# ziqin-h/GIVEPose

Measured on AMD Instinct MI355X. Metric: images/sec PoseNet fwd, bs=64 256x256 fp16, 1/2/4/8 MI355X; % MFMA roofline, higher is better.
Workload: dtype f16

## Files before the change

givepose_amd/_lib.py:

```python
import ctypes
import os
from ctypes import POINTER, Structure, c_char_p, c_double, c_float, c_int, c_long, c_void_p

_HERE = os.path.dirname(os.path.abspath(__file__))
LIB_PATH = os.environ.get("GP_LIB_PATH") or os.path.join(_HERE, "libgivepose_hip.so")

ABI_VERSION = 328
GP_F32, GP_F16, GP_F64 = 0, 1, 2
ACT_NONE, ACT_GELU, ACT_RELU, ACT_LRELU = 0, 1, 2, 3
EPI_NONE, EPI_GELU, EPI_RELU, EPI_LRELU, EPI_SCALE_RES, EPI_RES_RELU, EPI_LNFOLD_GELU = 0, 1, 2, 3, 4, 5, 6
ROT_6D, ROT_6D_Y, ROT_6D_Z, ROT_QUAT, ROT_EULER = 0, 1, 2, 3, 4
KC_GEMM, KC_DCNV3, KC_DWCONV_LN, KC_NORM, KC_ELEMENTWISE, KC_SMALL, KC_COUNT = 0, 1, 2, 3, 4, 5, 6
KC_NAMES = ["gemm", "dcnv3", "dwconv_ln", "norm", "elementwise", "small"]


class GemmDesc(Structure):
    _fields_ = [("X", c_void_p), ("W", c_void_p), ("bias", c_void_p), ("gamma", c_void_p), ("residual", c_void_p),
                ("C", c_void_p), ("workspace", c_void_p),
                ("M", c_int), ("N", c_int), ("K", c_int), ("ldx", c_int), ("ldc", c_int), ("ldres", c_int),
                ("epilogue", c_int), ("out_f32", c_int), ("splitk", c_int),
                ("B", c_int), ("H", c_int), ("Win", c_int), ("Cin", c_int), ("KH", c_int), ("KW", c_int),
                ("stride", c_int), ("pad", c_int), ("Ho", c_int), ("Wo", c_int), ("dtype", c_int),
                ("gn_partial", c_void_p), ("gn_groups", c_int), ("gn_hw", c_int), ("variant", c_int),
                ("ln_stats", c_void_p), ("ln_colsum", c_void_p), ("ln_nslab", c_int), ("ln_eps", c_float),
                ("co_scheduled", c_int), ("prefetch", c_void_p), ("prefetch_bytes", c_long),
                ("split_shift", c_int), ("x_plane_stride", c_long), ("w_plane_stride", c_long),
                ("out_planes", c_int), ("c_plane_stride", c_long),
                ("residual_f32", c_int), ("c16", c_void_p), ("ldc16", c_int), ("gn_rows", c_int)]


_P = c_void_p
PROTOTYPES = {
    "gp_last_error": ([], c_char_p),
    "gp_version": ([], c_int),
    "gp_device_info": ([POINTER(c_int), c_char_p, c_int], c_int),
    "gp_dcnv3_forward": ([_P, _P, _P, _P] + [c_int] * 9 + [c_float] + [c_int] * 7 + [_P], c_int),
    "gp_dcnv3_forward_any": ([_P] * 4 + [c_int] * 13 + [c_float] + [c_int] * 3 + [_P], c_int),
    "gp_dcnv3_backward": ([_P] * 7 + [c_long, c_long] + [c_int] * 13 + [c_float] + [c_int] * 3 + [_P], c_int),
    "gp_gemm": ([POINTER(GemmDesc), _P], c_int),
    "gp_gemm_gn_rows": ([c_int] * 4, c_int),
    "gp_split_planes": ([_P, _P, c_long, c_int, c_long, c_long, c_int, _P], c_int),
    "gp_convnext_mlp_pack_w2": ([_P, _P, c_int, _P], c_int),
    "gp_convnext_mlp_pack_w2_s32": ([_P, _P, c_int, _P], c_int),
# ... 115 lines not shown
```

givepose_amd/csrc/gemm.hip:

```cpp
#include "common.hpp"

namespace {

struct GemmKP {
    const void* X;
    const void* W;
    const float* bias;
    const float* gamma;
    const void* res;
    void* C;
    float* ws;
    int M, N, K, ldx, ldc, ldres, epi, out_f32;
    int conv, H, Win, Cin, KW, stride, pad, Ho, Wo;
    int tiles_m, tiles_n, nkt, kt_per_split, splitk;
    float* gn_partial;
    int gn_cpg, gn_hw;
    int early;
    const float* ln_stats;
    const float* ln_s;
    int ln_nsl;
    float ln_eps;
    int dbg;
    const char* pf;
    long pf_bytes;
    int split_n1;
    long xplane_b, wplane_b;
    float split_scale;
    int out_planes;
    long cplane;
    float split_up;
    void* c16;
    int ldc16;
};

__device__ __forceinline__ void clk_stamp(const GemmKP& p, int which) {
#ifdef GP_CLOCK_STAMPS
    if (threadIdx.x == 0 && p.ws && p.splitk <= 1) {
        __builtin_amdgcn_sched_barrier(0);
        const unsigned long long t = __builtin_amdgcn_s_memtime(), r = __builtin_amdgcn_s_memrealtime();
        unsigned long long* o = reinterpret_cast<unsigned long long*>(p.ws) + ((long)blockIdx.x * 2 + which) * 2;
        o[0] = t; o[1] = r;
        __builtin_amdgcn_sched_barrier(0);
    }
#endif
}

template <typename T>
// ... 363 lines not shown
        case GP_EPI_RELU: epilogue_generic<float, MT, NT, true, GP_EPI_RELU>(p, acc, slab, mb, nb, lane); break;
        case GP_EPI_LRELU: epilogue_generic<float, MT, NT, true, GP_EPI_LRELU>(p, acc, slab, mb, nb, lane); break;
        case GP_EPI_SCALE_RES: epilogue_generic<float, MT, NT, true, GP_EPI_SCALE_RES>(p, acc, slab, mb, nb, lane); break;
        case GP_EPI_RES_RELU: epilogue_generic<float, MT, NT, true, GP_EPI_RES_RELU>(p, acc, slab, mb, nb, lane); break;
        default: epilogue_generic<float, MT, NT, true, GP_EPI_NONE>(p, acc, slab, mb, nb, lane); break;
    }
}

template <typename T, int WM, int WN, int MT, int NT, int NS, bool DB = false, int RB = 128, bool PP = false, bool SPL = false, bool R32 = false>
__global__ __launch_bounds__(WM * WN * 64, WM * WN == 4 ? 2 : 1) void gemm_big_kernel(const GemmKP pin) {
    static_assert(NT == 4, "epilogue slab assumes a 64-wide wave tile");
    static_assert(!SPL || sizeof(T) == 2, "split-operand mode: fp16 planes");
    static_assert(!R32 || (sizeof(T) == 2 && !SPL), "R32: fp16 operands with an fp32 residual / output");
    typedef typename std::conditional<SPL || R32, float, T>::type RT;
    GemmKP p = pin;
    int kt0 = 0;
    if constexpr (!PP && !(DB && NS == 2)) {
        if (pin.splitk > 1) {
            kt0 = blockIdx.y * pin.kt_per_split;
            p.nkt = min(pin.nkt - kt0, pin.kt_per_split);
            p.C = reinterpret_cast<float*>(pin.C) + (long)blockIdx.y * pin.M * pin.N;
        }
    }
    static_assert(!PP || (WM * WN == 8 && (NS == 4 || NS == 5) && RB == 64 && !DB), "ping-pong schedule: 8 waves, 4/5-stage ring of 64-byte K steps");
    constexpr int NW = WM * WN;
    constexpr int BM = WM * MT * 16, BN = WN * NT * 16;
    static_assert(RB == 128 || (RB == 64 && !DB), "RB");
    constexpr int EPT = 16 / sizeof(T), KPT = RB / sizeof(T), CPR = RB / 16, RPI = 1024 / RB;
    constexpr int XI = BM / RPI / NW, WI = BN / RPI / NW;
    constexpr int STAGE = (BM + BN) * RB;
// ... 1129 lines not shown
    if (t < T) {
        tile(t, P1{}, std::true_type{});
        if constexpr (!GELU) activate(P0{});
        __builtin_amdgcn_sched_barrier(0);
        stores(t - 1);
        sync(t);
        clk_stamp(p, 1);
        activate(P1{});
    } else {
        clk_stamp(p, 1);
        activate(P0{});
    }
    stores(T - 1);
}

template <typename T, int WM, int WN, int MT, int NT, int NS, bool DB = false, int RB = 128, bool PP = false, bool SPL = false, bool R32 = false> void launch_big(GemmKP& p, hipStream_t s) {
    constexpr int BM = WM * MT * 16, BN = WN * NT * 16;
    p.nkt = p.K / (RB / (int)sizeof(T));
    if constexpr (SPL) { p.split_n1 = p.nkt; p.nkt *= 3; }
    p.tiles_m = cdiv(p.M, BM);
    p.tiles_n = cdiv(p.N, BN);
    int splits = 1;
    if constexpr (!PP && !(DB && NS == 2)) {
        if (p.splitk > 1) {
            if (p.splitk > p.nkt) p.splitk = p.nkt;
            p.kt_per_split = cdiv(p.nkt, p.splitk);
            p.splitk = cdiv(p.nkt, p.kt_per_split);
            splits = p.splitk;
        }
    }
    hipLaunchKernelGGL((gemm_big_kernel<T, WM, WN, MT, NT, NS, DB, RB, PP, SPL, R32>), dim3(p.tiles_m * p.tiles_n, splits), dim3(WM * WN * 64), 0, s, p);
}



__device__ __forceinline__ half8 to_mfma_lanes(half8 v, int pull) {
    pf_u32x4 u = __builtin_bit_cast(pf_u32x4, v);
#pragma unroll
    for (int d = 0; d < 4; ++d) u[d] = (unsigned)__builtin_amdgcn_ds_bpermute(pull, (int)u[d]);
    return __builtin_bit_cast(half8, u);
}

template <int MT, int NT, int KCH, bool CONV, bool GN>
__global__ __launch_bounds__(256) void gemm_smallm_kernel(const GemmKP p) {
    static_assert(!GN || NT == 2, "fused GroupNorm statistics: one workgroup = one (16 MT)-row chunk x 32 columns");
    extern __shared__ __attribute__((aligned(16))) char smallm_lds[];
    f32x4 (*red)[MT * NT][64] = reinterpret_cast<f32x4 (*)[MT * NT][64]>(smallm_lds);
    const int wave = threadIdx.x >> 6, lane = threadIdx.x & 63, r = lane & 15, q = lane >> 4;
    const int rl = lane >> 2, ql = lane & 3, pull = (4 * r + q) * 4;
    const int n0 = blockIdx.x * (16 * NT), m0 = blockIdx.y * (16 * MT);
    const int nk = p.K >> 5;
    const int per = (nk + 3) >> 2, k_lo = wave * per, k_hi = min(nk, k_lo + per);
    const PfSink pf = prefetch_issue(p, blockIdx.y * gridDim.x + blockIdx.x, gridDim.x * gridDim.y, wave, 4, lane);
    constexpr int TPW = (MT * NT + 3) / 4;
    f32x4 eb[TPW], eg[TPW];
    half4 er[TPW];
#pragma unroll
    for (int i = 0; i < TPW; ++i) {
        const int et = wave + 4 * i;
// ... 119 lines not shown
                const int b = m0 / p.gn_hw, ch = (m0 - b * p.gn_hw) / ROWS;
                float* o = p.gn_partial + (((long)b * cpi + ch) * G + (n0 + nt * 16 + qq * 4) / p.gn_cpg) * 2;
                if constexpr (MT == 1) {
                    o[0] = gred[nt][qq][0];
                    o[1] = gred[nt][qq][1];
                } else {
                    o[0] = gred[nt][qq][0] + gred[nt + 2][qq][0];
                    o[1] = gred[nt][qq][1] + gred[nt + 2][qq][1];
                }
            }
        }
    }
}

template <int MT, int NT, bool CONV, bool GN>
static void launch_smallm(const GemmKP& p, hipStream_t s) {
    constexpr int KMAX = (CONV && GN) ? (MT == 4 ? 6 : 9) : (CONV || MT + NT > 4) ? 9 : 16;
    const int per = (p.K / 32 + 3) / 4, rounds = (per + KMAX - 1) / KMAX, kch = (per + rounds - 1) / rounds;
    const dim3 grid(p.N / (16 * NT), (p.M + 16 * MT - 1) / (16 * MT));
    constexpr int LDS = 4 * MT * NT * 1024;
#define GP_SM(KCH)                                                                                                              \
    do {                                                                                                                        \
        auto kfn = gemm_smallm_kernel<MT, NT, (KCH) <= KMAX ? (KCH) : KMAX, CONV, GN>;                                          \
        if constexpr (LDS > 48 * 1024) {                                                                                        \
            static bool attr = false;                                                                                           \
            if (!attr) { (void)hipFuncSetAttribute((const void*)kfn, hipFuncAttributeMaxDynamicSharedMemorySize, LDS); attr = true; } \
        }                                                                                                                       \
        hipLaunchKernelGGL(kfn, grid, dim3(256), LDS, s, p);                                                                    \
    } while (0)
    if (kch <= 2) { GP_SM(2); return; }
    if (kch <= 4) { GP_SM(4); return; }
    if constexpr (!CONV) {
        if (kch <= 8) { GP_SM(8); return; }
    }
// ... 247 lines not shown
        GP_REQUIRE(d->Cin % KPT == 0, "gp_gemm: conv Cin=%d must be a multiple of %d", d->Cin, KPT);
        GP_REQUIRE(d->K == d->KH * d->KW * d->Cin, "gp_gemm: conv K=%d != KH*KW*Cin", d->K);
        GP_REQUIRE(d->KH * d->KW <= 32, "gp_gemm: at most 32 filter taps");
        const int Ho = (d->H + 2 * d->pad - d->KH) / d->stride + 1, Wo = (d->Win + 2 * d->pad - d->KW) / d->stride + 1;
        GP_REQUIRE(Ho == d->Ho && Wo == d->Wo, "gp_gemm: conv output %dx%d != expected %dx%d", d->Ho, d->Wo, Ho, Wo);
        GP_REQUIRE((long)d->B * Ho * Wo == d->M, "gp_gemm: conv M=%d != B*Ho*Wo", d->M);
        p.conv = 1; p.H = d->H; p.Win = d->Win; p.Cin = d->Cin; p.KW = d->KW; p.stride = d->stride; p.pad = d->pad;
        p.Ho = Ho; p.Wo = Wo;
    } else {
        GP_REQUIRE(d->ldx >= d->K && d->ldx % (16 / esz) == 0, "gp_gemm: ldx=%d invalid", d->ldx);
    }
    p.splitk = d->splitk > 1 ? d->splitk : 1;
    if (p.splitk > d->K / KPT * (split ? 3 : 1)) p.splitk = d->K / KPT * (split ? 3 : 1);
    if (p.splitk > 1) GP_REQUIRE(d->workspace != nullptr, "gp_gemm: splitk needs a workspace");
    hipStream_t s = (hipStream_t)stream;
    const double flops = 2.0 * d->M * d->N * d->K;
    const double xbytes = d->KH > 0 ? (double)d->B * d->H * d->Win * d->Cin * esz : (double)d->M * d->K * esz;
    const double bytes = xbytes + (double)d->N * d->K * esz + (double)d->M * d->N * (d->out_f32 ? 4 : esz) +
                         (d->epilogue >= GP_EPI_SCALE_RES ? (double)d->M * d->N * esz : 0.0);
    gp_timing_before(s, GP_KC_GEMM, flops, bytes);
    const bool wreg_ok = d->dtype == GP_F16 && d->KH == 0 && d->K == 512 && d->N % 256 == 0 && d->M % 32 == 0 && !d->out_f32 &&
                         p.splitk == 1 && !d->gn_partial && d->epilogue <= GP_EPI_LRELU && d->ldc % 4 == 0 &&
                         ((size_t)d->C & 7) == 0 && ((size_t)d->X & 15) == 0 && ((size_t)d->W & 15) == 0 &&
                         (!d->bias || ((size_t)d->bias & 15) == 0);
    const bool smallm_ok = d->dtype == GP_F16 && !split && !r32 && !d->c16 && d->epilogue != GP_EPI_LNFOLD_GELU &&
                           (!d->out_f32 || (d->epilogue <= GP_EPI_LRELU && !d->gn_partial && ((size_t)d->C & 15) == 0)) &&
                           (!d->gn_partial || (d->M % (d->gn_rows ? d->gn_rows : 64) == 0 && d->epilogue != GP_EPI_SCALE_RES && d->epilogue != GP_EPI_RES_RELU)) &&
                           d->N % 32 == 0 && (d->M % 16 == 0 || (d->KH == 0 && !d->gn_partial && d->M > 8)) && (d->KH == 0 || d->Cin % 32 == 0) && ((size_t)d->X & 15) == 0 &&
                           ((size_t)d->W & 15) == 0 && ((size_t)d->C & 7) == 0 && (!d->bias || ((size_t)d->bias & 15) == 0) &&
                           (!d->gamma || ((size_t)d->gamma & 15) == 0) && (!d->residual || ((size_t)d->residual & 7) == 0);
    int variant = d->variant % 100;
    p.dbg = d->variant / 100;
    p.early = wreg_early() ? 1 : 0;
    const bool gemv_ok = d->dtype == GP_F16 && !split && !r32 && !d->c16 && d->KH == 0 && !d->gn_partial && d->M <= 8 && d->K % 512 == 0 && d->N % 8 == 0 &&
                         d->ldx % 8 == 0 && d->epilogue <= GP_EPI_LRELU && ((size_t)d->X & 15) == 0 && ((size_t)d->W & 15) == 0 && ((size_t)d->C & 3) == 0 && d->ldc % 2 == 0;
    if (variant == 23 || (variant == 0 && gemv_ok && gemv_enabled())) {
        GP_REQUIRE(gemv_ok, "gp_gemm: variant 23 needs a plain fp16 GEMM of M <= 8 rows, K %% 512 == 0, N %% 8 == 0, bias / GELU / ReLU / LeakyReLU epilogue");
        p.splitk = 1;
        gp_timing_label("gemm v23 M%d N%d K%d epi%d", d->M, d->N, d->K, d->epilogue);
        const dim3 grid(d->N / 8);
        if (d->M <= 1) hipLaunchKernelGGL(gemv_kernel<1>, grid, dim3(256), 0, s, p);
        else if (d->M <= 2) hipLaunchKernelGGL(gemv_kernel<2>, grid, dim3(256), 0, s, p);
        else if (d->M <= 4) hipLaunchKernelGGL(gemv_kernel<4>, grid, dim3(256), 0, s, p);
        else hipLaunchKernelGGL(gemv_kernel<8>, grid, dim3(256), 0, s, p);
        GP_LAUNCH_CHECK("gp_gemm");
    }
    int sm_mt = 0;
    if (smallm_ok && smallm_enabled() && d->M <= smallm_max_rows()) {
        double best = 1e30;
        const int gn_mt = d->gn_partial ? (d->gn_rows ? d->gn_rows / 16 : 4) : 0;
        for (int mt = gn_mt ? gn_mt : 1; mt <= (gn_mt ? gn_mt : 4); mt *= 2) {
// ... 23 lines not shown
        }
        else variant = 4;
    }
    if (r32 && d->variant % 100 == 0 && variant != 10) variant = 7;
    const bool win_ok = d->dtype == GP_F16 && d->KH == 3 && d->KW == 3 && d->stride == 1 && d->pad == 1 && d->N == 256 &&
                        d->Cin % 32 == 0 && (d->Win == 64 || d->Win == 32 || d->Win == 16) && d->H % (256 / d->Win) == 0 &&
                        (!d->out_f32 || split) && p.splitk == 1 && d->ldc % 8 == 0 && ((size_t)d->C & 15) == 0 && !d->out_planes &&
                        (d->epilogue == GP_EPI_NONE || d->epilogue == GP_EPI_GELU || d->epilogue == GP_EPI_RELU);
    if (variant == 10 && d->variant % 100 == 0 && win_ok && conv_window_enabled()) variant = 13;
    GP_REQUIRE(!(d->gn_partial && d->gn_rows && d->gn_rows != 64) || variant == 18, "gp_gemm: gn_rows=%d needs the small-M kernel (variant 18: fp16, N %% 32 == 0, M %% gn_rows == 0), got variant %d", d->gn_rows, variant);
    GP_REQUIRE(((variant >= 2 && variant <= 13 && variant != 6) || (variant >= 16 && variant <= 22)) && (variant == 4 || p.splitk == 1), "gp_gemm: bad variant %d (split-K runs on variant 4)", variant);
    GP_REQUIRE(!split || variant == 4 || variant == 7 || variant == 8 || variant == 10 || variant == 13, "gp_gemm: split-operand mode runs on variants 4 / 7 / 8 / 10 / 13 (got %d)", variant);
    GP_REQUIRE(!r32 || variant == 7 || variant == 10, "gp_gemm: residual_f32 runs on variants 7 / 10 (got %d)", variant);
    GP_REQUIRE(!d->c16 || (variant != 13 && variant != 16 && variant != 17 && !split), "gp_gemm: c16 runs on the tile kernels (variants 2-5, 7-12), not on %d%s", variant, split ? " split" : "");
    if (d->KH > 0) gp_timing_label("conv%dx%d s%d v%d %dx%d Cin%d Cout%d M%d%s%s", d->KH, d->KW, d->stride, variant, d->H, d->Win, d->Cin, d->N, d->M, d->gn_partial ? (d->gn_rows == 16 ? " +gn16" : d->gn_rows == 32 ? " +gn32" : " +gn") : "", split ? " split3" : "");
    else gp_timing_label("gemm v%d M%d N%d K%d epi%d%s%s%s", variant, d->M, d->N, d->K, d->epilogue, p.splitk > 1 ? " splitK" : "", d->gn_partial ? " +gn" : "", split ? " split3" : "");
    if (variant == 18) {
        GP_REQUIRE(smallm_ok, "gp_gemm: variant 18 needs a plain fp16 GEMM / conv (fp16 out, no split-K), N %% 32 == 0, M %% 16 == 0 (%% 64 with fused GroupNorm statistics)");
        GP_REQUIRE(d->M / (16 * sm_mt) <= 65535, "gp_gemm: variant 18: M=%d gives more than 65535 row tiles (grid.y)", d->M);
        if (d->gn_partial) {
            GP_REQUIRE(sm_mt == 1 || sm_mt == 2 || sm_mt == 4, "gp_gemm: variant 18: bad statistics chunk");
            if (d->KH > 0) { if (sm_mt == 4) launch_smallm<4, 2, true, true>(p, s); else if (sm_mt == 2) launch_smallm<2, 2, true, true>(p, s); else launch_smallm<1, 2, true, true>(p, s); }
            else { if (sm_mt == 4) launch_smallm<4, 2, false, true>(p, s); else if (sm_mt == 2) launch_smallm<2, 2, false, true>(p, s); else launch_smallm<1, 2, false, true>(p, s); }
        }
        else if (d->KH > 0) { if (sm_mt == 4) launch_smallm<4, 2, true, false>(p, s); else if (sm_mt == 2) launch_smallm<2, 2, true, false>(p, s); else launch_smallm<1, 2, true, false>(p, s); }
        else { if (sm_mt == 4) launch_smallm<4, 2, false, false>(p, s); else if (sm_mt == 2) launch_smallm<2, 2, false, false>(p, s); else launch_smallm<1, 2, false, false>(p, s); }
        GP_LAUNCH_CHECK("gp_gemm");
    }
    if (variant == 16) {
        GP_REQUIRE(wreg_ok, "gp_gemm: variant 16 needs a plain fp16 GEMM with K = 512, N %% 256 == 0, M %% 32 == 0, epilogue none/gelu/relu/lrelu");
        const int nsl = d->N / 256, tiles = d->M / 32;
        const int want = gp_num_cus() / nsl > 0 ? gp_num_cus() / nsl : 1;
        p.tiles_m = cdiv(tiles, want);
        const int groups = cdiv(tiles, p.tiles_m);
        const int grid = cdiv(groups * nsl, 8) * 8;
        switch (d->epilogue) {
            case GP_EPI_GELU:
#ifdef GP_WREG_STAMPS
                if (p.dbg == 16 && p.ws) { hipLaunchKernelGGL((gemm_wreg_kernel<GP_EPI_GELU, 16>), dim3(grid), dim3(512), 0, s, p); break; }
                if (p.dbg == 1) { hipLaunchKernelGGL((gemm_wreg_kernel<GP_EPI_GELU, 1>), dim3(grid), dim3(512), 0, s, p); break; }
                if (p.dbg == 2) { hipLaunchKernelGGL((gemm_wreg_kernel<GP_EPI_GELU, 2>), dim3(grid), dim3(512), 0, s, p); break; }
// ... 83 lines not shown
        if (d->dtype == GP_F16) launch_big<half_t, 2, 4, 4, 4, 4, false, 64, true>(p, s); else launch_big<float, 2, 2, 4, 4, 2>(p, s);
        GP_LAUNCH_CHECK("gp_gemm");
    }
    if (variant == 8) {
        if (split) launch_big<half_t, 2, 2, 8, 4, 3, false, 64, false, true>(p, s);
        else if (d->dtype == GP_F16) launch_big<half_t, 2, 2, 8, 4, 3, false, 64>(p, s); else launch_big<float, 2, 2, 4, 4, 2>(p, s);
        GP_LAUNCH_CHECK("gp_gemm");
    }
    if (variant == 9) {
        if (d->dtype == GP_F16) launch_big<half_t, 2, 2, 8, 4, 4, false, 64>(p, s); else launch_big<float, 2, 2, 4, 4, 2>(p, s);
        GP_LAUNCH_CHECK("gp_gemm");
    }
    if (variant == 7) {
        if (split) launch_big<half_t, 2, 2, 4, 4, 2, true, 128, false, true>(p, s);
        else if (r32) launch_big<half_t, 2, 2, 4, 4, 2, true, 128, false, false, true>(p, s);
        else if (d->dtype == GP_F16) launch_big<half_t, 2, 2, 4, 4, 2, true>(p, s); else launch_big<float, 2, 2, 4, 4, 2>(p, s);
        GP_LAUNCH_CHECK("gp_gemm");
    }
    if (variant == 5) {
        if (d->dtype == GP_F16) launch_big<half_t, 2, 2, 4, 4, 4>(p, s); else launch_big<float, 2, 2, 4, 4, 4>(p, s);
        GP_LAUNCH_CHECK("gp_gemm");
    }
    if (variant == 4) {
        if (p.splitk > 1) {
            GemmKP q = p;
            q.C = d->workspace; q.out_f32 = 1; q.ldc = d->N; q.epi = GP_EPI_NONE; q.bias = nullptr; q.gamma = nullptr; q.res = nullptr;
            if (split) launch_big<half_t, 2, 2, 4, 4, 2, false, 128, false, true>(q, s);
            else if (d->dtype == GP_F16) launch_big<half_t, 2, 2, 4, 4, 2>(q, s); else launch_big<float, 2, 2, 4, 4, 2>(q, s);
            p.splitk = q.splitk;
            const long work = (long)d->M * (d->N / 4);
            if (d->dtype == GP_F16 && !split) hipLaunchKernelGGL(splitk_reduce_kernel<half_t>, dim3(cdiv(work, 256)), dim3(256), 0, s, p);
// ... 18 lines not shown
```

givepose_amd/csrc/norm.hip:

```cpp
#include "common.hpp"

#ifdef GP_DW_STAMPS
__device__ unsigned long long gp_dw_stamp_buf[8 * 16];
extern "C" int gp_dw_stamps_read(unsigned long long* host) {
    return hipMemcpyFromSymbol(host, HIP_SYMBOL(gp_dw_stamp_buf), sizeof(unsigned long long) * 8 * 16) == hipSuccess ? 0 : 1;
}
#define GP_DW_MARK(k) do { if (blockIdx.x == gridDim.x / 2 + 1 && blockIdx.y == 0) { const unsigned long long t__ = __builtin_amdgcn_s_memtime(); if ((threadIdx.x & 63) == 0) gp_dw_stamp_buf[(threadIdx.x >> 6) * 16 + (k)] = t__; } } while (0)
__device__ unsigned long long gp_dwt_stamp_buf[8 * 64];
extern "C" int gp_dwt_stamps_read(unsigned long long* host) {
    return hipMemcpyFromSymbol(host, HIP_SYMBOL(gp_dwt_stamp_buf), sizeof(unsigned long long) * 8 * 64) == hipSuccess ? 0 : 1;
}
#define GP_DWT_MARK(k) do { if (blockIdx.x == gridDim.x / 2 + 1) { const unsigned long long t__ = __builtin_amdgcn_s_memtime(); if ((threadIdx.x & 63) == 0) gp_dwt_stamp_buf[(threadIdx.x >> 6) * 64 + (k)] = t__; } } while (0)
#else
#define GP_DW_MARK(k) do { } while (0)
#define GP_DWT_MARK(k) do { } while (0)
#endif
namespace {

template <int NV>
__device__ __forceinline__ void pixel_group_sum(float (&v)[NV], int CT, float* red) {
    if (CT <= 64) {
#pragma unroll
        for (int i = 0; i < NV; ++i) v[i] = group_sum(v[i], CT);
    } else {
// ... 155 lines not shown
        if (pix0 + p >= n_pixels) break;
        const float rstd = rsqrtf(v[p] * invC + eps);
        Vec16<T> o;
#pragma unroll
        for (int e = 0; e < VEC; ++e) {
            const float val = acc[p][e] * rstd * gw[e] + gb[e];
            o.set(e, act == GP_ACT_GELU ? gelu_for<T>(val) : apply_act(val, act));
        }
        store16p<T>(y, (pix0 + p) * C + cs * VEC, o, pl);
    }
}

template <int TH>
__global__ __launch_bounds__(256) void dwconv3_ln_tile_kernel(const half_t* __restrict__ x, const half_t* __restrict__ wt, const float* __restrict__ bias,
                                                              const float* __restrict__ lnw, const float* __restrict__ lnb, half_t* __restrict__ y,
                                                              int H, int W, float eps) {
    constexpr int C = 256, HR = TH + 2, HC = 18, PPT = 2 * TH, SPR = 16 / PPT;
    extern __shared__ __attribute__((aligned(16))) char dw3_lds[];
    const int t = threadIdx.x, o = t & 31, slot = t >> 5, r = slot / SPR, ch = slot % SPR;
    const int tpr = W >> 4;
    const int rb = blockIdx.x / tpr, c0 = (blockIdx.x - rb * tpr) * 16;
    const long row0 = (long)rb * TH;
    const int h0 = (int)(row0 % H);
    const half_t* xim = x + (row0 - h0) * W * C;
    constexpr int NPC = HR * HC * 32, NIT = (NPC + 255) / 256;
    uint4 pc[NIT];
#pragma unroll
    for (int k = 0; k < NIT; ++k) {
        const int i = t + 256 * k, px = i >> 5, hr = px / HC, hc = px - hr * HC;
        const int hi = h0 - 1 + hr, wi = c0 - 1 + hc;
        pc[k] = (i < NPC && (unsigned)hi < (unsigned)H && (unsigned)wi < (unsigned)W)
                    ? *reinterpret_cast<const uint4*>(xim + ((long)hi * W + wi) * C + (i & 31) * 8) : uint4{0u, 0u, 0u, 0u};
    }
    Vec16<half_t> wv[9];
#pragma unroll
    for (int k = 0; k < 9; ++k) wv[k] = load16<half_t>(wt + k * C + o * 8);
    float acc[PPT][8];
    {
        float bv[8];
// ... 1599 lines not shown
extern "C" int gp_dwconv_ln_groups(const void* x, const void* wt, const float* bias, const float* ln_w, const float* ln_b, void* y, int B,
                                   int H, int W, int C, int KS, float eps, int act, const int* crop_group_start, int dtype, void* stream) {
    GP_REQUIRE(x && wt && bias && ln_w && ln_b && y && crop_group_start, "gp_dwconv_ln_groups: null pointer");
    GP_REQUIRE(dtype == GP_F32 || dtype == GP_F16, "gp_dwconv_ln_groups: bad dtype");
    const int esz = dtype == GP_F16 ? 2 : 4;
    GP_REQUIRE(ct_ok(C, esz) && C / (16 / esz) >= 16, "gp_dwconv_ln_groups: unsupported C=%d", C);
    GP_REQUIRE(KS == 3 || KS == 7, "gp_dwconv_ln_groups: KS=%d unsupported (3 or 7)", KS);
    GP_REQUIRE(B > 0 && W % 16 == 0 && H % 2 == 0 && x != y, "gp_dwconv_ln_groups: B=%d, W=%d %% 16, H=%d %% 2, y != x required", B, W, H);
    GP_REQUIRE(act == GP_ACT_NONE || act == GP_ACT_GELU || act == GP_ACT_RELU || act == GP_ACT_LRELU, "gp_dwconv_ln_groups: bad act");
    const long n_pixels = (long)B * H * W / 4;
    const int CT = C / (16 / esz), PG = 256 / CT;
    const long strips = (n_pixels + 7) / 8;
    hipStream_t s = (hipStream_t)stream;
    gp_timing_before(s, GP_KC_DWCONV_LN, 2.0 * n_pixels * C * KS * KS, (double)n_pixels * C * esz * 2);
    gp_timing_label("dwconv%d_ln groups C%d %dx%d B%d", KS, C, H, W, B);
    const bool narrow = dtype == GP_F16 && (cdiv(strips, PG) < dw_narrow_below() || (KS == 3 && dw3_narrow_always()));
    dim3 grid(narrow ? cdiv((n_pixels + 1) / 2, PG) : cdiv(strips, PG));
#define GP_DWG(T, K, P) hipLaunchKernelGGL((dwconv_ln_kernel<T, K, P>), grid, dim3(256), 0, s, (const T*)x, (const T*)wt, bias, ln_w, ln_b, (T*)y, H, W, C, eps, act, n_pixels, 0l, crop_group_start)
    if (dtype == GP_F16) {
        if (narrow) { if (KS == 7) GP_DWG(half_t, 7, 2); else GP_DWG(half_t, 3, 2); }
        else { if (KS == 7) GP_DWG(half_t, 7, 8); else GP_DWG(half_t, 3, 8); }
    }
    else { if (KS == 7) GP_DWG(float, 7, 8); else GP_DWG(float, 3, 8); }
#undef GP_DWG
    GP_LAUNCH_CHECK("gp_dwconv_ln_groups");
}

extern "C" int gp_dwconv7_raw_stats(const void* x, const void* wt, const float* bias, void* y, float* stats, int B, int H,
                                    int W, int C, int dtype, void* stream) {
    GP_REQUIRE(x && wt && bias && y && stats, "gp_dwconv7_raw_stats: null pointer");
// ... 144 lines not shown
```

givepose_amd/ops.py:

```python
import ctypes
import os

import torch

from . import _lib
from ._lib import (ACT_GELU, ACT_LRELU, ACT_NONE, ACT_RELU, EPI_GELU, EPI_LNFOLD_GELU, EPI_LRELU, EPI_NONE, EPI_RELU, EPI_RES_RELU,
                   EPI_SCALE_RES, GP_F16, GP_F32, GP_F64, GemmDesc, check)

__all__ = ["dtype_code", "gemm", "conv2d_nhwc", "dcnv3_forward", "dcnv3_backward", "dcnv3_forward_into", "dcnv3_xyz_project", "convnext_stem", "dwconv_ln",
           "layernorm", "groupnorm", "upsample_bilinear2x", "deconv_col2im", "xyz_out_layer", "pointwise_k3",
           "pnp_conv1", "pnp_conv1_masked", "pool_mmm", "xyz_conv3x3_s2", "size_head", "pose_tail", "pose_tail_rt", "mask_resize_nearest"]


def _L():
    return _lib.load()


def _stream():
    return ctypes.c_void_p(torch.cuda.current_stream().cuda_stream)


def dtype_code(dt):
    if dt == torch.float16:
        return GP_F16
# ... 94 lines not shown
CO_SCHEDULED = False


def auto_splitk(M, N, K, esz, n_cu=256, plain=True):
    tiles = ((M + 127) // 128) * ((N + 127) // 128)
    nkt = K // (128 // esz)
    if plain and esz == 2 and K >= 4096 and 32 < tiles <= 128:
        return 4
    if tiles >= 32 or nkt < 32:
        return 1
    return max(1, min(nkt // 4, (n_cu + tiles - 1) // tiles, 32))


def gemm(x, w, out, bias=None, epilogue=EPI_NONE, gamma=None, residual=None, M=None, K=None, ldx=None, ldc=None,
         ldres=None, conv=None, splitk=None, variant=0, gn=None, ln=None, prefetch=None, _stamps=None, x_planes=False,
         out_planes=False, out16=None):
    split = isinstance(w, SplitW)
    dt = x.dtype
    if split:
        _chk(x, "x", torch.float32), _chk(out, "out", torch.float32)
        if residual is not None:
            _chk(residual, "residual", torch.float32)
        code = GP_F16
    else:
        code = dtype_code(dt)
        _chk(x, "x"), _chk(w, "w", dt), _chk(out, "out")
    N = w.shape[0]
    Kw = w.shape[1]
    d = GemmDesc()
    if conv is not None:
        B, H, W_, Cin, KH, KW, stride, pad = (conv[k] for k in ("B", "H", "W", "Cin", "KH", "KW", "stride", "pad"))
# ... 48 lines not shown
    elif _stamps is not None:
        d.workspace = _stamps.data_ptr()
    d.M, d.N, d.K, d.ldx, d.ldc = M, N, K, ldx, ldc
    d.ldres = (residual.stride(0) if ldres is None else ldres) if residual is not None else 0
    if not split and residual is not None and residual.dtype == torch.float32 and dt == torch.float16:
        if out.dtype != torch.float32:
            raise TypeError("gemm: an fp32 residual goes with an fp32 output")
        d.residual_f32 = 1
        splitk = 1
    if out16 is not None:
        if out16.dtype != torch.float16 or out.dtype != torch.float32 or dt != torch.float16 or split:
            raise TypeError("gemm(out16): fp16 operands, float32 out, float16 out16")
        d.c16, d.ldc16 = out16.data_ptr(), out16.stride(0)
        splitk = 1
    d.epilogue, d.out_f32, d.splitk, d.dtype, d.variant = epilogue, out_f32, splitk, code, variant
    d.co_scheduled = 1 if CO_SCHEDULED else 0
    if prefetch is not None:
        d.prefetch, d.prefetch_bytes = prefetch.data_ptr(), prefetch.numel() * prefetch.element_size()
    if ln is not None:
        d.ln_stats, d.ln_colsum, d.ln_nslab, d.ln_eps = ln[0].data_ptr(), ln[1].data_ptr(), ln[2], ln[3]
    if gn is not None:
        d.gn_partial, d.gn_groups, d.gn_hw = gn[0].data_ptr(), gn[1], gn[2]
        d.gn_rows = gn[3] if len(gn) > 3 else 0
    check(_L().gp_gemm(ctypes.byref(d), _stream()), "gp_gemm")
    return out


def conv2d_nhwc(x, w_packed, KH, KW, stride, pad, out=None, bias=None, epilogue=EPI_NONE, variant=0, gn=None,
                residual=None, prefetch=None, x_planes=False, out16=None):
    B, H, W_, Cin = x.shape
# ... 334 lines not shown
```

givepose_amd/posenet.py:

```python
import ctypes
import os
from collections import OrderedDict

import numpy as np
import torch
import torch.nn as nn

from . import _lib, ops, synth
from ._lib import (ACT_GELU, ACT_RELU, EPI_GELU, EPI_LNFOLD_GELU, EPI_LRELU, EPI_NONE, EPI_SCALE_RES)
from .config import FLAT_OPS, ROT_TYPES, PoseNetConfig, validate

OM_LD = 128


def enc0_xyz_pack(sd, prefix="nocs_encoder.features.0.", dtype=torch.float32):
    f64 = lambda k: sd[prefix + k].detach().to(device="cpu", dtype=torch.float64)
    cw, cb = f64("conv.weight").reshape(256, -1), f64("conv.bias")
    iw, ib = f64("dcnv3.input_proj.weight"), f64("dcnv3.input_proj.bias")
    ow, ob = f64("dcnv3.output_proj.weight"), f64("dcnv3.output_proj.bias")
    fold = torch.cat([iw @ cw, (iw @ cb + ib)[:, None]], 1)
    m = torch.cat([ow[:, 64 * g:64 * g + 64] @ fold[64 * g:64 * g + 64] for g in range(4)], 1)
    return m.to(dtype).contiguous(), ob.to(dtype).contiguous()


# ... 300 lines not shown
            buf["a_pos"] = self._packed["att.pos"].to(T).repeat(B, 1).contiguous()
        buf["feat_cat"] = e(B, 8, 8, 512)
        if cfg.pnp_head == "att":
            buf["p_patch"], buf["p_x"], buf["p_h"] = e(B * 64, 320), e(B * 64, 192), e(B * 64, 192)
            buf["p_qkv"], buf["p_att"], buf["p_mlp"], buf["p_flat"] = e(B * 64, 576), e(B * 64, 192), e(B * 64, 768), e(B * 64, 192)
            buf["p_pos"] = self._packed["apn.pos"].to(T).repeat(B, 1).contiguous()
        else:
            buf["p0"], buf["p1"], buf["p2"] = e(B, 32, 32, 128), e(B, 16, 16, 128), e(B, 8, 8, 128)
        buf["fc1"] = e(B, 2048)
        buf["hh"], buf["hz"] = f(B, 256), f(B, 256)
        if FLAT_OPS[cfg.flat_op]:
            buf["pooled"] = e(B, 128 * FLAT_OPS[cfg.flat_op])
        buf["pred_rot"], buf["pred_t"], buf["rot_allo"], buf["rot_ego"], buf["trans"] = f(B, cfg.rot_dim), f(B, 3), f(B, 9), f(B, 9), f(B, 3)
        buf["rot6d"] = buf["pred_rot"] if cfg.rot_dim == 6 else None
        plan = {"buf": buf, "graph": None, "warm": False, "ragged": bool(ragged), "enc0_xyz": enc0_xyz}
        if ragged:
            buf["grp"] = torch.arange(B, dtype=torch.int32, device=device)
            buf["grp_host"] = torch.arange(B, dtype=torch.int32).pin_memory()
            for k in ("roi_img", "roi_mask", "roi_coord_2d", "bbox_center", "mean_size"):
                buf[k].zero_()
            buf["roi_wh"].fill_(1.0)
            buf["resize_ratio"].fill_(1.0)
            buf["cam_K"].copy_(torch.eye(3, device=device).expand(B, 3, 3))
        self._plans[key] = plan
        self._evict_plans(key)
        return plan

    def _gn(self, x, w, b, act, buf, G=32, out=None, ldy=None, fused=False, out_planes=False, rows=64):
        B = x.shape[0]
        C = x.shape[-1]
# ... 166 lines not shown
                if plan.get("ragged"):
                    if li == 0:
                        ops.pointwise_k3(buf["nocs_nhwc4"], W[q + "conv_w"], W[q + "conv_b"], xin.view(-1, 256))
                    else:
                        ops.gemm(prev.view(-1, 256), W[q + "conv_w"], xin.view(-1, 256), bias=W[q + "conv_b"])
                    ops.dwconv_ln_groups(xin, W[q + "dw_w"], W[q + "dw_b"], W[q + "ln_w"], W[q + "ln_b"], buf[f"e_x1{li}"], 3, buf["grp"], act=ACT_GELU)
                    ops.gemm(buf[f"e_x1{li}"], W[q + "om_w"], buf[f"e_om{li}"], bias=W[q + "om_b"])
                    if not xyz0:
                        ops.dcnv3_forward_into(buf[f"e_proj{li}"], buf[f"e_om{li}"], buf[f"e_om{li}"][:, 72:], buf[f"e_g{li}"], 3, 2, 1, 1, 4, 64, 1.0,
                                               off_ld=OM_LD, mask_ld=OM_LD, mask_is_logits=True)
                Bg = self.dcn_couple if (self.dcn_couple and B > self.dcn_couple) else B
                if plan.get("ragged"):
                    Bg = B + 1
                if B % Bg and not plan.get("ragged"):
                    raise ValueError(f"batch {B} is not a multiple of dcn_couple = {Bg}")
                for g0 in range(0, B if not plan.get("ragged") else 0, Bg):
                    gs = slice(g0, g0 + Bg)
                    nq = Bg * ro * ro
                    npre = min(Bg * r * r, (nq + r + 8 + 15) // 16 * 16)
                    xin_g = xin[gs]
                    if li == 0:
                        ops.pointwise_k3(buf["nocs_nhwc4"][g0 * r * r:][:npre], W[q + "conv_w"], W[q + "conv_b"], xin_g.view(-1, 256)[:npre])
                    else:
                        ops.gemm(prev[gs].view(-1, 256)[:npre], W[q + "conv_w"], xin_g.view(-1, 256)[:npre], bias=W[q + "conv_b"])
                    x1_g = buf[f"e_x1{li}"][g0 * r * r // 4:(g0 + Bg) * r * r // 4]
                    om_g = buf[f"e_om{li}"][g0 * r * r // 4:(g0 + Bg) * r * r // 4]
                    ops.dwconv_ln(xin_g, W[q + "dw_w"], W[q + "dw_b"], W[q + "ln_w"], W[q + "ln_b"], x1_g, 3, act=ACT_GELU, n_pixels=nq)
                    ops.gemm(x1_g, W[q + "om_w"], om_g, bias=W[q + "om_b"])
                    if not xyz0:
                        ops.dcnv3_forward_into(buf[f"e_proj{li}"][gs], om_g, om_g[:, 72:], buf[f"e_g{li}"][gs], 3, 2, 1, 1, 4, 64, 1.0,
                                               off_ld=OM_LD, mask_ld=OM_LD, mask_is_logits=True)
# ... 260 lines not shown
```

include/givepose_hip.h:

```cpp
#ifndef GIVEPOSE_HIP_H
#define GIVEPOSE_HIP_H

#ifdef __cplusplus
extern "C" {
#endif

enum gp_status { GP_OK = 0, GP_ERR_INVALID = -1, GP_ERR_LAUNCH = -2, GP_ERR_RUNTIME = -3 };
enum gp_dtype { GP_F32 = 0, GP_F16 = 1, GP_F64 = 2  };
#define GP_OUT_PLANES 0x100
#define GP_IN_F32 0x200
#define GP_SPLIT_SHIFT 11
enum gp_act { GP_ACT_NONE = 0, GP_ACT_GELU = 1, GP_ACT_RELU = 2, GP_ACT_LRELU = 3  };
enum gp_epilogue {
    GP_EPI_NONE = 0,
    GP_EPI_GELU = 1,
    GP_EPI_RELU = 2,
    GP_EPI_LRELU = 3,
    GP_EPI_SCALE_RES = 4,
    GP_EPI_RES_RELU = 5,
    GP_EPI_LNFOLD_GELU = 6
};

const char* gp_last_error(void);
#define GP_ABI_VERSION 328
int gp_version(void);
int gp_device_info(int* cu_count, char* arch, int arch_len);

int gp_dcnv3_forward(const void* in, const void* offset, const void* mask, void* out, int N, int H, int W,
                     int G, int D, int K, int stride, int pad, int dil, float offset_scale,
                     int remove_center, int im2col_step, int off_ld, int mask_ld, int mask_is_logits,
                     int dtype, int om_dtype, void* stream);

int gp_dcnv3_forward_any(const void* in, const void* offset, const void* mask, void* out, int N, int H, int W, int G,
                         int D, int kernel_h, int kernel_w, int stride_h, int stride_w, int pad_h, int pad_w,
                         int dilation_h, int dilation_w, float offset_scale, int remove_center, int im2col_step,
                         int dtype, void* stream);

int gp_dcnv3_backward(const void* in, const void* offset, const void* mask, const void* grad_out, void* grad_in,
                      void* grad_offset, void* grad_mask, long offset_numel, long mask_numel, int N, int H, int W, int G,
// ... 22 lines not shown
    const float* ln_stats;
    const float* ln_colsum;
    int ln_nslab;
    float ln_eps;
    int co_scheduled;
    const void* prefetch;
    long prefetch_bytes;
    int split_shift;
    long x_plane_stride, w_plane_stride;
    int out_planes;
    long c_plane_stride;
    int residual_f32;
    void* c16;
    int ldc16;
    int gn_rows;
} gp_gemm_desc;
int gp_gemm_gn_rows(int M, int N, int K, int hw);
int gp_gemm(const gp_gemm_desc* d, void* stream);

int gp_split_planes(const float* x, void* planes, long rows, int cols, long ldx, long plane_stride, int split_shift,
                    void* stream);

int gp_convnext_mlp_pack_w2(const void* w2, void* w2p, int C, void* stream);
int gp_convnext_mlp_pack_w2_s32(const void* w2, void* w2p, int C, void* stream);
#define GP_MLP_S32 0x400
int gp_convnext_mlp(const void* x, const void* w1, const float* b1, const void* w2p, const float* b2,
                    const float* gamma, const void* residual, void* out, long M, int C, int dtype, void* stream);

int gp_convnext_stem(const float* img, const float* w, const float* b, const float* ln_w, const float* ln_b,
                     void* out, int B, int H, int W, int C0, float eps, int dtype, void* stream);
// ... 137 lines not shown
```

Measured before the change: 12820.

## Batch encoder DCN groups into segmented GEMM and grouped dwconv launches

```diff
diff --git a/givepose_amd/_lib.py b/givepose_amd/_lib.py
--- a/givepose_amd/_lib.py
+++ b/givepose_amd/_lib.py
@@ -5,7 +5,7 @@
 _HERE = os.path.dirname(os.path.abspath(__file__))
 LIB_PATH = os.environ.get("GP_LIB_PATH") or os.path.join(_HERE, "libgivepose_hip.so")
 
-ABI_VERSION = 328
+ABI_VERSION = 329
 GP_F32, GP_F16, GP_F64 = 0, 1, 2
 ACT_NONE, ACT_GELU, ACT_RELU, ACT_LRELU = 0, 1, 2, 3
 EPI_NONE, EPI_GELU, EPI_RELU, EPI_LRELU, EPI_SCALE_RES, EPI_RES_RELU, EPI_LNFOLD_GELU = 0, 1, 2, 3, 4, 5, 6
@@ -26,7 +26,8 @@
                 ("co_scheduled", c_int), ("prefetch", c_void_p), ("prefetch_bytes", c_long),
                 ("split_shift", c_int), ("x_plane_stride", c_long), ("w_plane_stride", c_long),
                 ("out_planes", c_int), ("c_plane_stride", c_long),
-                ("residual_f32", c_int), ("c16", c_void_p), ("ldc16", c_int), ("gn_rows", c_int)]
+                ("residual_f32", c_int), ("c16", c_void_p), ("ldc16", c_int), ("gn_rows", c_int),
+                ("seg_count", c_int), ("seg_stride_rows", c_long)]
 
 
 _P = c_void_p
diff --git a/givepose_amd/csrc/gemm.hip b/givepose_amd/csrc/gemm.hip
--- a/givepose_amd/csrc/gemm.hip
+++ b/givepose_amd/csrc/gemm.hip
@@ -31,6 +31,7 @@
     float split_up;
     void* c16;
     int ldc16;
+    long seg_x, seg_c, seg_r;
 };
 
 __device__ __forceinline__ void clk_stamp(const GemmKP& p, int which) {
@@ -424,6 +425,11 @@
     static_assert(!R32 || (sizeof(T) == 2 && !SPL), "R32: fp16 operands with an fp32 residual / output");
     typedef typename std::conditional<SPL || R32, float, T>::type RT;
     GemmKP p = pin;
+    if constexpr (sizeof(T) == 2 && DB && NS == 2 && !PP && !SPL && !R32) {
+        p.X = reinterpret_cast<const char*>(pin.X) + (long)blockIdx.z * pin.seg_x;
+        p.C = reinterpret_cast<char*>(pin.C) + (long)blockIdx.z * pin.seg_c;
+        if (pin.res) p.res = reinterpret_cast<const char*>(pin.res) + (long)blockIdx.z * pin.seg_r;
+    }
     int kt0 = 0;
     if constexpr (!PP && !(DB && NS == 2)) {
         if (pin.splitk > 1) {
@@ -1583,7 +1589,7 @@
     stores(T - 1);
 }
 
-template <typename T, int WM, int WN, int MT, int NT, int NS, bool DB = false, int RB = 128, bool PP = false, bool SPL = false, bool R32 = false> void launch_big(GemmKP& p, hipStream_t s) {
+template <typename T, int WM, int WN, int MT, int NT, int NS, bool DB = false, int RB = 128, bool PP = false, bool SPL = false, bool R32 = false> void launch_big(GemmKP& p, hipStream_t s, int segs = 1) {
     constexpr int BM = WM * MT * 16, BN = WN * NT * 16;
     p.nkt = p.K / (RB / (int)sizeof(T));
     if constexpr (SPL) { p.split_n1 = p.nkt; p.nkt *= 3; }
@@ -1598,7 +1604,7 @@
             splits = p.splitk;
         }
     }
-    hipLaunchKernelGGL((gemm_big_kernel<T, WM, WN, MT, NT, NS, DB, RB, PP, SPL, R32>), dim3(p.tiles_m * p.tiles_n, splits), dim3(WM * WN * 64), 0, s, p);
+    hipLaunchKernelGGL((gemm_big_kernel<T, WM, WN, MT, NT, NS, DB, RB, PP, SPL, R32>), dim3(p.tiles_m * p.tiles_n, splits, segs), dim3(WM * WN * 64), 0, s, p);
 }
 
 
@@ -1611,7 +1617,13 @@
 }
 
 template <int MT, int NT, int KCH, bool CONV, bool GN>
-__global__ __launch_bounds__(256) void gemm_smallm_kernel(const GemmKP p) {
+__global__ __launch_bounds__(256) void gemm_smallm_kernel(const GemmKP pin) {
+    GemmKP p = pin;
+    if constexpr (!CONV && !GN) {
+        p.X = reinterpret_cast<const char*>(pin.X) + (long)blockIdx.z * pin.seg_x;
+        p.C = reinterpret_cast<char*>(pin.C) + (long)blockIdx.z * pin.seg_c;
+        if (pin.res) p.res = reinterpret_cast<const char*>(pin.res) + (long)blockIdx.z * pin.seg_r;
+    }
     static_assert(!GN || NT == 2, "fused GroupNorm statistics: one workgroup = one (16 MT)-row chunk x 32 columns");
     extern __shared__ __attribute__((aligned(16))) char smallm_lds[];
     f32x4 (*red)[MT * NT][64] = reinterpret_cast<f32x4 (*)[MT * NT][64]>(smallm_lds);
@@ -1761,10 +1773,10 @@
 }
 
 template <int MT, int NT, bool CONV, bool GN>
-static void launch_smallm(const GemmKP& p, hipStream_t s) {
+static void launch_smallm(const GemmKP& p, hipStream_t s, int segs = 1) {
     constexpr int KMAX = (CONV && GN) ? (MT == 4 ? 6 : 9) : (CONV || MT + NT > 4) ? 9 : 16;
     const int per = (p.K / 32 + 3) / 4, rounds = (per + KMAX - 1) / KMAX, kch = (per + rounds - 1) / rounds;
-    const dim3 grid(p.N / (16 * NT), (p.M + 16 * MT - 1) / (16 * MT));
+    const dim3 grid(p.N / (16 * NT), (p.M + 16 * MT - 1) / (16 * MT), segs);
     constexpr int LDS = 4 * MT * NT * 1024;
 #define GP_SM(KCH)                                                                                                              \
     do {                                                                                                                        \
@@ -2042,10 +2054,19 @@
     if (p.splitk > d->K / KPT * (split ? 3 : 1)) p.splitk = d->K / KPT * (split ? 3 : 1);
     if (p.splitk > 1) GP_REQUIRE(d->workspace != nullptr, "gp_gemm: splitk needs a workspace");
     hipStream_t s = (hipStream_t)stream;
-    const double flops = 2.0 * d->M * d->N * d->K;
+    const int segs = d->seg_count > 1 ? d->seg_count : 1;
+    if (segs > 1) {
+        const long osz = d->out_f32 ? 4 : esz;
+        GP_REQUIRE(d->dtype == GP_F16 && d->KH == 0 && !split && !r32 && !d->c16 && !d->gn_partial && p.splitk == 1 && d->epilogue != GP_EPI_LNFOLD_GELU,
+                   "gp_gemm: row segments need a plain fp16 GEMM (no conv, split-K, split-operand mode, fused GroupNorm, LNFOLD, fp32 residual, c16)");
+        GP_REQUIRE(segs <= 65535 && d->seg_stride_rows >= d->M, "gp_gemm: row segments: seg_count=%d (<= 65535), seg_stride_rows=%ld (>= M=%d)", segs, d->seg_stride_rows, d->M);
+        p.seg_x = d->seg_stride_rows * d->ldx * esz; p.seg_c = d->seg_stride_rows * d->ldc * osz; p.seg_r = d->residual ? d->seg_stride_rows * d->ldres * esz : 0;
+        GP_REQUIRE(p.seg_x % 16 == 0 && p.seg_c % 16 == 0 && p.seg_r % 16 == 0, "gp_gemm: row segments: segment bases must keep 16-byte alignment");
+    }
+    const double flops = 2.0 * d->M * d->N * d->K * segs;
     const double xbytes = d->KH > 0 ? (double)d->B * d->H * d->Win * d->Cin * esz : (double)d->M * d->K * esz;
-    const double bytes = xbytes + (double)d->N * d->K * esz + (double)d->M * d->N * (d->out_f32 ? 4 : esz) +
-                         (d->epilogue >= GP_EPI_SCALE_RES ? (double)d->M * d->N * esz : 0.0);
+    const double bytes = xbytes * segs + (double)d->N * d->K * esz + (double)d->M * d->N * (d->out_f32 ? 4 : esz) * segs +
+                         (d->epilogue >= GP_EPI_SCALE_RES ? (double)d->M * d->N * esz * segs : 0.0);
     gp_timing_before(s, GP_KC_GEMM, flops, bytes);
     const bool wreg_ok = d->dtype == GP_F16 && d->KH == 0 && d->K == 512 && d->N % 256 == 0 && d->M % 32 == 0 && !d->out_f32 &&
                          p.splitk == 1 && !d->gn_partial && d->epilogue <= GP_EPI_LRELU && d->ldc % 4 == 0 &&
@@ -2062,7 +2083,8 @@
     p.early = wreg_early() ? 1 : 0;
     const bool gemv_ok = d->dtype == GP_F16 && !split && !r32 && !d->c16 && d->KH == 0 && !d->gn_partial && d->M <= 8 && d->K % 512 == 0 && d->N % 8 == 0 &&
                          d->ldx % 8 == 0 && d->epilogue <= GP_EPI_LRELU && ((size_t)d->X & 15) == 0 && ((size_t)d->W & 15) == 0 && ((size_t)d->C & 3) == 0 && d->ldc % 2 == 0;
-    if (variant == 23 || (variant == 0 && gemv_ok && gemv_enabled())) {
+    if (variant == 23 || (variant == 0 && gemv_ok && gemv_enabled() && segs == 1)) {
+        GP_REQUIRE(segs == 1, "gp_gemm: row segments run on variants 7 / 18, not on 23");
         GP_REQUIRE(gemv_ok, "gp_gemm: variant 23 needs a plain fp16 GEMM of M <= 8 rows, K %% 512 == 0, N %% 8 == 0, bias / GELU / ReLU / LeakyReLU epilogue");
         p.splitk = 1;
         gp_timing_label("gemm v23 M%d N%d K%d epi%d", d->M, d->N, d->K, d->epilogue);
@@ -2116,6 +2138,10 @@
     GP_REQUIRE(!r32 || variant == 7 || variant == 10, "gp_gemm: residual_f32 runs on variants 7 / 10 (got %d)", variant);
     GP_REQUIRE(!d->c16 || (variant != 13 && variant != 16 && variant != 17 && !split), "gp_gemm: c16 runs on the tile kernels (variants 2-5, 7-12), not on %d%s", variant, split ? " split" : "");
     if (d->KH > 0) gp_timing_label("conv%dx%d s%d v%d %dx%d Cin%d Cout%d M%d%s%s", d->KH, d->KW, d->stride, variant, d->H, d->Win, d->Cin, d->N, d->M, d->gn_partial ? (d->gn_rows == 16 ? " +gn16" : d->gn_rows == 32 ? " +gn32" : " +gn") : "", split ? " split3" : "");
+    else if (segs > 1) {
+        GP_REQUIRE(variant == 7 || variant == 18, "gp_gemm: row segments run on variants 7 / 18 (this shape takes %d)", variant);
+        gp_timing_label("gemm v%d M%d N%d K%d epi%d seg%d", variant, d->M, d->N, d->K, d->epilogue, segs);
+    }
     else gp_timing_label("gemm v%d M%d N%d K%d epi%d%s%s%s", variant, d->M, d->N, d->K, d->epilogue, p.splitk > 1 ? " splitK" : "", d->gn_partial ? " +gn" : "", split ? " split3" : "");
     if (variant == 18) {
         GP_REQUIRE(smallm_ok, "gp_gemm: variant 18 needs a plain fp16 GEMM / conv (fp16 out, no split-K), N %% 32 == 0, M %% 16 == 0 (%% 64 with fused GroupNorm statistics)");
@@ -2126,7 +2152,7 @@
             else { if (sm_mt == 4) launch_smallm<4, 2, false, true>(p, s); else if (sm_mt == 2) launch_smallm<2, 2, false, true>(p, s); else launch_smallm<1, 2, false, true>(p, s); }
         }
         else if (d->KH > 0) { if (sm_mt == 4) launch_smallm<4, 2, true, false>(p, s); else if (sm_mt == 2) launch_smallm<2, 2, true, false>(p, s); else launch_smallm<1, 2, true, false>(p, s); }
-        else { if (sm_mt == 4) launch_smallm<4, 2, false, false>(p, s); else if (sm_mt == 2) launch_smallm<2, 2, false, false>(p, s); else launch_smallm<1, 2, false, false>(p, s); }
+        else { if (sm_mt == 4) launch_smallm<4, 2, false, false>(p, s, segs); else if (sm_mt == 2) launch_smallm<2, 2, false, false>(p, s, segs); else launch_smallm<1, 2, false, false>(p, s, segs); }
         GP_LAUNCH_CHECK("gp_gemm");
     }
     if (variant == 16) {
@@ -2240,7 +2266,7 @@
     if (variant == 7) {
         if (split) launch_big<half_t, 2, 2, 4, 4, 2, true, 128, false, true>(p, s);
         else if (r32) launch_big<half_t, 2, 2, 4, 4, 2, true, 128, false, false, true>(p, s);
-        else if (d->dtype == GP_F16) launch_big<half_t, 2, 2, 4, 4, 2, true>(p, s); else launch_big<float, 2, 2, 4, 4, 2>(p, s);
+        else if (d->dtype == GP_F16) launch_big<half_t, 2, 2, 4, 4, 2, true>(p, s, segs); else launch_big<float, 2, 2, 4, 4, 2>(p, s);
         GP_LAUNCH_CHECK("gp_gemm");
     }
     if (variant == 5) {
diff --git a/givepose_amd/csrc/norm.hip b/givepose_amd/csrc/norm.hip
--- a/givepose_amd/csrc/norm.hip
+++ b/givepose_amd/csrc/norm.hip
@@ -193,15 +193,20 @@
 template <int TH>
 __global__ __launch_bounds__(256) void dwconv3_ln_tile_kernel(const half_t* __restrict__ x, const half_t* __restrict__ wt, const float* __restrict__ bias,
                                                               const float* __restrict__ lnw, const float* __restrict__ lnb, half_t* __restrict__ y,
-                                                              int H, int W, float eps) {
+                                                              int H, int W, float eps, const int* __restrict__ grp = nullptr) {
     constexpr int C = 256, HR = TH + 2, HC = 18, PPT = 2 * TH, SPR = 16 / PPT;
     extern __shared__ __attribute__((aligned(16))) char dw3_lds[];
     const int t = threadIdx.x, o = t & 31, slot = t >> 5, r = slot / SPR, ch = slot % SPR;
     const int tpr = W >> 4;
     const int rb = blockIdx.x / tpr, c0 = (blockIdx.x - rb * tpr) * 16;
     const long row0 = (long)rb * TH;
-    const int h0 = (int)(row0 % H);
-    const half_t* xim = x + (row0 - h0) * W * C;
+    long src0 = row0;
+    if (grp) {
+        const int q = H >> 2, c = (int)(row0 / q);
+        src0 += 3l * min(max(grp[c], 0), c) * q;
+    }
+    const int h0 = (int)(src0 % H);
+    const half_t* xim = x + (src0 - h0) * W * C;
     constexpr int NPC = HR * HC * 32, NIT = (NPC + 255) / 256;
     uint4 pc[NIT];
 #pragma unroll
@@ -1831,6 +1836,20 @@
     hipStream_t s = (hipStream_t)stream;
     gp_timing_before(s, GP_KC_DWCONV_LN, 2.0 * n_pixels * C * KS * KS, (double)n_pixels * C * esz * 2);
     gp_timing_label("dwconv%d_ln groups C%d %dx%d B%d", KS, C, H, W, B);
+    {
+        const int th3 = dw3_tile_rows();
+        if (KS == 3 && dtype == GP_F16 && C == 256 && act == GP_ACT_GELU && H % (4 * th3) == 0 && n_pixels / 64 >= dw3_tile_min()) {
+            static bool attr_set = false;
+            if (!attr_set) {
+                (void)hipFuncSetAttribute((const void*)dwconv3_ln_tile_kernel<4>, hipFuncAttributeMaxDynamicSharedMemorySize, 6 * 18 * 512);
+                (void)hipFuncSetAttribute((const void*)dwconv3_ln_tile_kernel<2>, hipFuncAttributeMaxDynamicSharedMemorySize, 4 * 18 * 512);
+                attr_set = true;
+            }
+            if (th3 == 4) hipLaunchKernelGGL(dwconv3_ln_tile_kernel<4>, dim3((unsigned)(n_pixels / 64)), dim3(256), 6 * 18 * 512, s, (const half_t*)x, (const half_t*)wt, bias, ln_w, ln_b, (half_t*)y, H, W, eps, crop_group_start);
+            else hipLaunchKernelGGL(dwconv3_ln_tile_kernel<2>, dim3((unsigned)(n_pixels / 32)), dim3(256), 4 * 18 * 512, s, (const half_t*)x, (const half_t*)wt, bias, ln_w, ln_b, (half_t*)y, H, W, eps, crop_group_start);
+            GP_LAUNCH_CHECK("gp_dwconv_ln_groups");
+        }
+    }
     const bool narrow = dtype == GP_F16 && (cdiv(strips, PG) < dw_narrow_below() || (KS == 3 && dw3_narrow_always()));
     dim3 grid(narrow ? cdiv((n_pixels + 1) / 2, PG) : cdiv(strips, PG));
 #define GP_DWG(T, K, P) hipLaunchKernelGGL((dwconv_ln_kernel<T, K, P>), grid, dim3(256), 0, s, (const T*)x, (const T*)wt, bias, ln_w, ln_b, (T*)y, H, W, C, eps, act, n_pixels, 0l, crop_group_start)
diff --git a/givepose_amd/ops.py b/givepose_amd/ops.py
--- a/givepose_amd/ops.py
+++ b/givepose_amd/ops.py
@@ -132,7 +132,23 @@
 
 def gemm(x, w, out, bias=None, epilogue=EPI_NONE, gamma=None, residual=None, M=None, K=None, ldx=None, ldc=None,
          ldres=None, conv=None, splitk=None, variant=0, gn=None, ln=None, prefetch=None, _stamps=None, x_planes=False,
-         out_planes=False, out16=None):
+         out_planes=False, out16=None, segments=None, _segs=None):
+    if segments is not None and segments[0] > 1:
+        count, stride_rows = int(segments[0]), int(segments[1])
+        if M is None or conv is not None or isinstance(w, SplitW) or gn is not None or ln is not None or out16 is not None:
+            raise RuntimeError("gemm(segments): a plain GEMM with an explicit M")
+        if stride_rows < M or min(x.shape[0], out.shape[0]) < (count - 1) * stride_rows + M:
+            raise RuntimeError(f"gemm(segments): {count} segments of {M} rows, {stride_rows} apart, do not fit x / out")
+        kw = dict(bias=bias, epilogue=epilogue, gamma=gamma, M=M, K=K, ldx=ldx, ldc=ldc, ldres=ldres, splitk=splitk, variant=variant, prefetch=prefetch)
+        if x.dtype == torch.float16:
+            try:
+                return gemm(x, w, out, residual=residual, _segs=(count, stride_rows), **kw)
+            except _lib.GivePoseHipError as e:
+                if "row segments" not in str(e):
+                    raise
+        for g in range(count):
+            gemm(x[g * stride_rows:], w, out[g * stride_rows:], residual=None if residual is None else residual[g * stride_rows:], **kw)
+        return out
     split = isinstance(w, SplitW)
     dt = x.dtype
     if split:
@@ -211,6 +227,8 @@
         d.c16, d.ldc16 = out16.data_ptr(), out16.stride(0)
         splitk = 1
     d.epilogue, d.out_f32, d.splitk, d.dtype, d.variant = epilogue, out_f32, splitk, code, variant
+    if _segs is not None:
+        d.seg_count, d.seg_stride_rows = _segs
     d.co_scheduled = 1 if CO_SCHEDULED else 0
     if prefetch is not None:
         d.prefetch, d.prefetch_bytes = prefetch.data_ptr(), prefetch.numel() * prefetch.element_size()
diff --git a/givepose_amd/posenet.py b/givepose_amd/posenet.py
--- a/givepose_amd/posenet.py
+++ b/givepose_amd/posenet.py
@@ -338,6 +338,10 @@
         buf["pred_rot"], buf["pred_t"], buf["rot_allo"], buf["rot_ego"], buf["trans"] = f(B, cfg.rot_dim), f(B, 3), f(B, 9), f(B, 9), f(B, 3)
         buf["rot6d"] = buf["pred_rot"] if cfg.rot_dim == 6 else None
         plan = {"buf": buf, "graph": None, "warm": False, "ragged": bool(ragged), "enc0_xyz": enc0_xyz}
+        if (not ragged and self.dcn_couple and B > self.dcn_couple and B % self.dcn_couple == 0 and T == torch.float16 and (B <= 256 or B % 256 == 0)
+                and cfg.nocsmap_encoder == "conv" and cfg.use_dcn == "dcnv3" and os.environ.get("GP_ENC_GROUP_TABLE") != "0"):
+            plan["enc_group_table"] = True
+            buf["grp"] = (torch.arange(B, dtype=torch.int32, device=device) // self.dcn_couple) * self.dcn_couple
         if ragged:
             buf["grp"] = torch.arange(B, dtype=torch.int32, device=device)
             buf["grp_host"] = torch.arange(B, dtype=torch.int32).pin_memory()
@@ -534,7 +538,17 @@
                     Bg = B + 1
                 if B % Bg and not plan.get("ragged"):
                     raise ValueError(f"batch {B} is not a multiple of dcn_couple = {Bg}")
-                for g0 in range(0, B if not plan.get("ragged") else 0, Bg):
+                if plan.get("enc_group_table") and li > 0 and only_layer is None:
+                    if Bg % min(Bg, 256):
+                        raise RuntimeError(f"gp_dcnv3_forward: batch({Bg}) must divide im2col_step({min(Bg, 256)})")
+                    npre = min(Bg * r * r, (Bg * ro * ro + r + 8 + 15) // 16 * 16)
+                    ops.gemm(prev.view(-1, 256), W[q + "conv_w"], xin.view(-1, 256), bias=W[q + "conv_b"], M=npre, segments=(B // Bg, Bg * r * r))
+                    ops.dwconv_ln_groups(xin, W[q + "dw_w"], W[q + "dw_b"], W[q + "ln_w"], W[q + "ln_b"], buf[f"e_x1{li}"], 3, buf["grp"], act=ACT_GELU)
+                    ops.gemm(buf[f"e_x1{li}"], W[q + "om_w"], buf[f"e_om{li}"], bias=W[q + "om_b"])
+                    ops.dcnv3_forward_into(buf[f"e_proj{li}"], buf[f"e_om{li}"], buf[f"e_om{li}"][:, 72:], buf[f"e_g{li}"], 3, 2, 1, 1, 4, 64, 1.0,
+                                           off_ld=OM_LD, mask_ld=OM_LD, mask_is_logits=True)
+                    Bg = B + 1
+                for g0 in range(0, B if not plan.get("ragged") and Bg <= B else 0, Bg):
                     gs = slice(g0, g0 + Bg)
                     nq = Bg * ro * ro
                     npre = min(Bg * r * r, (nq + r + 8 + 15) // 16 * 16)
diff --git a/include/givepose_hip.h b/include/givepose_hip.h
--- a/include/givepose_hip.h
+++ b/include/givepose_hip.h
@@ -22,7 +22,7 @@
 };
 
 const char* gp_last_error(void);
-#define GP_ABI_VERSION 328
+#define GP_ABI_VERSION 329
 int gp_version(void);
 int gp_device_info(int* cu_count, char* arch, int arch_len);
 
@@ -75,6 +75,8 @@
     void* c16;
     int ldc16;
     int gn_rows;
+    int seg_count;
+    long seg_stride_rows;
 } gp_gemm_desc;
 int gp_gemm_gn_rows(int M, int N, int K, int hw);
 int gp_gemm(const gp_gemm_desc* d, void* stream);
```

After: 12850, median of 3. No clear change (+0.2%).
